# cscott/compressjs

Hardware: NVIDIA H100
Metric: bzip2_-9_encode_MBps (higher is better)
Workload: dtype u8

## Files before the change

compressjs_b200/csrc/huff.cu:

```cuda
#include "enc.h"
#include "huffalloc.cuh"

#define HF_THREADS 256
#define HF_TILE_GROUPS 256
#define HF_TILE_BYTES (HF_TILE_GROUPS * HUFF_GROUP)
#define HF_TILE_VEC (HF_TILE_BYTES / 16)
#define HF_TILE_REGS ((HF_TILE_VEC + HF_THREADS - 1) / HF_THREADS)
#define HF_COPIES 16
#define HF_EVEN 0x01F07C1Fu

struct HuffSmem {
  u8 tile[HF_TILE_BYTES + 16];
  u16 cost[SEL_STRIDE];
  u8 sel[SEL_STRIDE];
  u32 tbl[HUFF_MAXSYM][HF_COPIES];
  u32 freq[HUFF_MAXGROUPS][HUFF_MAXSYM + 2];
  int work[HUFF_MAXGROUPS][HUFF_MAXSYM + 2];
  u32 skey[HUFF_MAXGROUPS][HUFF_MAXSYM + 2];
  u16 order[HUFF_MAXGROUPS][HUFF_MAXSYM + 2];
  u8 len[HUFF_MAXGROUPS][HUFF_MAXSYM + 6];
  u32 chist[1024];
  u32 ws[HF_THREADS / 32 + 1];
  u32 gcount[HUFF_MAXGROUPS];
  u32 misc[8];
};

template <class S>
__device__ void pack_lengths(S& s, u32 ntab, u32 A) {
  for (u32 i = threadIdx.x; i < A * HF_COPIES; i += HF_THREADS) {
    const u32 sym = i / HF_COPIES;
    u32 p = 0;
    for (u32 t = 0; t < ntab; t++) p |= (u32)s.len[t][sym] << (5 * t);
    s.tbl[sym][i % HF_COPIES] = p;
  }
  __syncthreads();
}

__device__ void build_tables(HuffSmem& s, u32 ntab, u32 A) {
  const u32 tid = threadIdx.x;
  for (u32 i = tid; i < ntab * A; i += HF_THREADS) {
    const u32 t = i / A, sym = i % A;
    s.skey[t][sym] = (s.freq[t][sym] << 9) | sym;
  }
  __syncthreads();
  for (u32 i = tid; i < ntab * A; i += HF_THREADS) {
    const u32 t = i / A, sym = i % A;
    const u32 k = s.skey[t][sym];
    u32 r = 0;
    for (u32 j = 0; j < A; j++) r += (s.skey[t][j] < k) ? 1u : 0u;
    s.order[t][r] = (u16)sym;
    s.work[t][r] = (int)(k >> 9);
  }
  __syncthreads();
  if (tid < ntab) ha_allocate(s.work[tid], (int)A, 20);
  __syncthreads();
  for (u32 i = tid; i < ntab * A; i += HF_THREADS) {
    const u32 t = i / A, r = i % A;
    s.len[t][s.order[t][r]] = (u8)s.work[t][r];
  }
  __syncthreads();
  pack_lengths(s, ntab, A);
}

struct TileRegs {
  uint4 r[HF_TILE_REGS];
  unsigned long long hm;
};
__device__ __forceinline__ void tile_fetch(TileRegs& t, const u8* nar, const unsigned long long* hmask, u32 g0, u32 nsel, bool any_hi) {
  const uint4* src = reinterpret_cast<const uint4*>(nar + (size_t)g0 * HUFF_GROUP);
#pragma unroll
  for (int k = 0; k < HF_TILE_REGS; k++) {
    const u32 i = k * HF_THREADS + threadIdx.x;
    if (i < HF_TILE_VEC) t.r[k] = __ldg(src + i);
  }
  t.hm = any_hi && g0 + threadIdx.x < nsel ? __ldg(hmask + g0 + threadIdx.x) : 0ull;
}
__device__ __forceinline__ void tile_store(const TileRegs& t, u8* tile) {
#pragma unroll
  for (int k = 0; k < HF_TILE_REGS; k++) {
    const u32 i = k * HF_THREADS + threadIdx.x;
    if (i < HF_TILE_VEC) reinterpret_cast<uint4*>(tile)[i] = t.r[k];
  }
}

template <class F>
__device__ __forceinline__ void for_group(const u8* tile, u32 cnt, unsigned long long hm, F f) {
  const u32 base = threadIdx.x * HUFF_GROUP;
  if (cnt == HUFF_GROUP && hm == 0) {
    const u32* wp = reinterpret_cast<const u32*>(tile + (base & ~3u));
    const u32 sh = (base & 2u) * 8u;
    u32 nxt = wp[0];
#pragma unroll
    for (u32 k = 0; k < 13; k++) {
      const u32 cur = nxt;
      nxt = wp[k + 1];
      const u32 w = __funnelshift_r(cur, nxt, sh);
      f(w & 0xffu);
      f((w >> 8) & 0xffu);
      if (k < 12) {
        f((w >> 16) & 0xffu);
        f(w >> 24);
      }
    }
  } else {
    for (u32 j = 0; j < cnt; j++) f((u32)tile[base + j] | (u32)((hm >> j) & 1u) << 8);
  }
}

template <class S>
__device__ __forceinline__ void assign_selectors(S& s, const u8* nar, const unsigned long long* hmask, u32 m, u32 nsel, u32 ntab,
                                                 bool any_hi) {
  const u32 tid = threadIdx.x, lane = tid % HF_COPIES;
  TileRegs tr;
  tile_fetch(tr, nar, hmask, 0, nsel, any_hi);
  for (u32 g0 = 0; g0 < nsel; g0 += HF_TILE_GROUPS) {
    tile_store(tr, s.tile);
    const unsigned long long hm = tr.hm;
    __syncthreads();
    if (g0 + HF_TILE_GROUPS < nsel) tile_fetch(tr, nar, hmask, g0 + HF_TILE_GROUPS, nsel, any_hi);
    const u32 g = g0 + tid;
    if (g < nsel) {
      const u32 cnt = min(50u, m - 50u * g);
      u32 ae = 0, ao = 0;
      for_group(s.tile, cnt, hm, [&](u32 sy) {
        const u32 v = s.tbl[sy][lane];
        ae += v & HF_EVEN;
        ao += (v >> 5) & HF_EVEN;
      });
      const u32 c[HUFF_MAXGROUPS] = {ae & 1023u, ao & 1023u, (ae >> 10) & 1023u, (ao >> 10) & 1023u, ae >> 20, ao >> 20};
      u32 best = 0, bc = c[0];
#pragma unroll
      for (u32 t = 1; t < HUFF_MAXGROUPS; t++)
        if (t < ntab && c[t] < bc) { best = t; bc = c[t]; }
      s.sel[g] = (u8)best;
      s.cost[g] = (u16)bc;
    }
    __syncthreads();
  }
}

template <class S>
__device__ __forceinline__ void recount(S& s, const u8* nar, const unsigned long long* hmask, u32 m, u32 nsel, u32 ntab, bool any_hi) {
  const u32 tid = threadIdx.x;
  for (u32 i = tid; i < ntab * (HUFF_MAXSYM + 2); i += HF_THREADS) (&s.freq[0][0])[i] = 0;
  TileRegs tr;
  tile_fetch(tr, nar, hmask, 0, nsel, any_hi);
  __syncthreads();
  for (u32 g0 = 0; g0 < nsel; g0 += HF_TILE_GROUPS) {
    tile_store(tr, s.tile);
    const unsigned long long hm = tr.hm;
    __syncthreads();
    if (g0 + HF_TILE_GROUPS < nsel) tile_fetch(tr, nar, hmask, g0 + HF_TILE_GROUPS, nsel, any_hi);
    const u32 g = g0 + tid;
    if (g < nsel) {
      u32* f = s.freq[s.sel[g]];
      for_group(s.tile, min(50u, m - 50u * g), hm, [&](u32 sy) { atomicAdd(&f[sy], 1u); });
    }
    __syncthreads();
  }
}

__device__ __forceinline__ u32 mtf6_find(u32 list, u32 v) {
  u32 j = 0;
#pragma unroll
  for (u32 k = 1; k < HUFF_MAXGROUPS; k++) j = (((list >> (4 * k)) & 15u) == v) ? k : j;
  return j;
}
__device__ __forceinline__ u32 mtf6_front(u32 list, u32 j) {
  const u32 v = (list >> (4 * j)) & 15u;
  const u32 low = list & ((1u << (4 * j)) - 1u);
  const u32 high = list & ~((1u << (4 * (j + 1))) - 1u);
  return high | (low << 4) | v;
}
__device__ __forceinline__ u32 rec_apply(u32 R, u32 v) {
  u32 cnt = R >> 28, lst = R & 0x00ffffffu, j = cnt;
#pragma unroll
  for (u32 k = 0; k < HUFF_MAXGROUPS; k++) j = (k < cnt && ((lst >> (4 * k)) & 15u) == v) ? k : j;
  if (j == cnt) {
    lst = ((lst << 4) | v) & 0x00ffffffu;
    cnt++;
  } else {
    const u32 low = lst & ((1u << (4 * j)) - 1u);
    const u32 high = lst & ~((1u << (4 * (j + 1))) - 1u);
    lst = high | (low << 4) | v;
  }
  return (cnt << 28) | lst;
}
__device__ __forceinline__ bool rec_has(u32 R, u32 v) {
  const u32 cnt = R >> 28;
  bool f = false;
#pragma unroll
  for (u32 k = 0; k < HUFF_MAXGROUPS; k++) f = f || (k < cnt && ((R >> (4 * k)) & 15u) == v);
  return f;
}
__device__ __forceinline__ u32 rec_op(u32 A, u32 B) {
  u32 cnt = B >> 28, lst = B & 0x00ffffffu;
  const u32 ca = A >> 28;
#pragma unroll
  for (u32 k = 0; k < HUFF_MAXGROUPS; k++) {
    const u32 v = (A >> (4 * k)) & 15u;
    if (k < ca && !rec_has(B, v)) { lst |= v << (4 * cnt); cnt++; }
  }
  return (cnt << 28) | lst;
}
__device__ __forceinline__ u32 rec_full(u32 R) {
  u32 cnt = R >> 28, lst = R & 0x00ffffffu;
#pragma unroll
  for (u32 v = 0; v < HUFF_MAXGROUPS; v++)
    if (!rec_has(R, v)) { lst |= v << (4 * cnt); cnt++; }
  return lst;
}

template <class S>
__device__ void write_block(S& s, u32 blk, u32 m, u32 alpha, u32 nsel, u32 ng, const u32* __restrict__ used, u8* __restrict__ sel_out,
                            u8* __restrict__ selmtf_out, HuffBlk* __restrict__ hb, u32* __restrict__ goff_out) {
  const u32 tid = threadIdx.x, A = alpha + 2;
  unsigned long long bits;
  {
    const u32 w = tid >> 5, lane = tid & 31;
    const u32 per = (nsel + HF_THREADS / 32 - 1) / (HF_THREADS / 32);
    const u32 ga = min(nsel, w * per), gb = min(nsel, ga + per);
    u32 part = 0;
    for (u32 g = ga + lane; g < gb; g += 32) part += s.cost[g];
    part = warp_reduce_add(part);
    if (lane == 0) s.ws[w] = part;
    __syncthreads();
    u32 carry = 0, total = 0;
    for (u32 i = 0; i < HF_THREADS / 32; i++) {
      const u32 x = s.ws[i];
      carry += i < w ? x : 0u;
      total += x;
    }
    u32* go = goff_out + (size_t)blk * SEL_STRIDE;
    for (u32 g0 = ga; g0 < gb; g0 += 32) {
      const u32 g = g0 + lane;
      const u32 c = g < gb ? (u32)s.cost[g] : 0u;
      const u32 inc = warp_incl_add(c);
      if (g < gb) go[g] = carry + inc - c;
      carry += __shfl_sync(FULL_MASK, inc, 31);
    }
    if (tid == 0) go[nsel] = total;
    bits = total;
    __syncthreads();
  }
  u8* so = sel_out + (size_t)blk * SEL_STRIDE;
  for (u32 g = tid; g < nsel; g += HF_THREADS) so[g] = s.sel[g];
  for (u32 i = tid; i < ng * A; i += HF_THREADS) hb->len[i / A][i % A] = s.len[i / A][i % A];
  u32 selbits = 0;
  {
    const u32 per = (nsel + HF_THREADS - 1) / HF_THREADS;
    const u32 ga = min(nsel, tid * per), gb = min(nsel, ga + per);
    u32 P = 0;
    for (u32 g = ga; g < gb; g++) P = rec_apply(P, s.sel[g]);
    u32* sa = s.chist;
    u32* sb = s.chist + HF_THREADS;
    sa[tid] = P;
    __syncthreads();
    u32 *src = sa, *dst = sb;
    for (u32 o = 1; o < HF_THREADS; o <<= 1) {
      u32 x = src[tid];
      if (tid >= o) x = rec_op(src[tid - o], x);
      dst[tid] = x;
      __syncthreads();
      u32* tmp = src; src = dst; dst = tmp;
    }
    u32 L = rec_full(tid ? src[tid - 1] : 0u);
    u8* sm = selmtf_out + (size_t)blk * SEL_STRIDE;
    for (u32 g = ga; g < gb; g++) {
      const u32 j = mtf6_find(L, s.sel[g]);
      L = mtf6_front(L, j);
      sm[g] = (u8)j;
      selbits += j + 1;
    }
    __syncthreads();
  }
  {
    unsigned long long b2 = selbits;
    __shared__ unsigned long long red2[HF_THREADS / 32];
    for (int o = 16; o > 0; o >>= 1) b2 += __shfl_xor_sync(FULL_MASK, b2, o);
    if ((tid & 31) == 0) red2[tid >> 5] = b2;
    __syncthreads();
    b2 = 0;
    for (int i = 0; i < HF_THREADS / 32; i++) b2 += red2[i];
    bits += b2;
  }
  if (tid == 0) {
    unsigned long long hbits = 48 + 32 + 1 + 24 + 16 + 3 + 15;
    for (u32 r = 0; r < 16; r++) {
      const u32 w = used[blk * 8 + (r >> 1)];
      if ((w >> ((r & 1) * 16)) & 0xffffu) hbits += 16;
    }
    for (u32 t = 0; t < ng; t++) {
      hbits += 5;
      u32 cur = s.len[t][0];
      for (u32 i = 0; i < A; i++) {
        const u32 l = s.len[t][i];
        hbits += 2 * (l > cur ? l - cur : cur - l) + 1;
        cur = l;
      }
    }
    hb->ngroups = ng; hb->nsel = nsel; hb->alpha = alpha; hb->m = m;
    hb->body_bits = hbits + bits;
  }
}

__global__ void __launch_bounds__(HF_THREADS, 2)
k_huffman(const u8* __restrict__ sym_lo, const unsigned long long* __restrict__ sym_hi, const u32* __restrict__ any_hi_arr,
          const u32* __restrict__ m_arr, const u32* __restrict__ freq0, const u32* __restrict__ used, u8* __restrict__ sel_out,
          u8* __restrict__ selmtf_out, HuffBlk* __restrict__ hb_out, u32* __restrict__ goff_out) {
  extern __shared__ __align__(16) unsigned char smem_raw[];
  HuffSmem& s = *reinterpret_cast<HuffSmem*>(smem_raw);
  const u32 tid = threadIdx.x;
  const u32 blk = blockIdx.x;
  const u32 m = m_arr[blk];
  HuffBlk* hb = hb_out + blk;
  if (m == 0) {
    if (tid == 0) { hb->ngroups = 0; hb->nsel = 0; hb->alpha = 0; hb->m = 0; hb->body_bits = 0; }
    return;
  }
  u32 alpha = 0;
  for (int k = 0; k < 8; k++) alpha += __popc(used[blk * 8 + k]);
  const u32 A = alpha + 2;
  const u32 nsel = (m + HUFF_GROUP - 1) / HUFF_GROUP;
  const u8* nar = sym_lo + ((size_t)blk << SEG_SHIFT);
  const unsigned long long* hmask = sym_hi + (size_t)blk * SEL_STRIDE;
  const bool any_hi = any_hi_arr[blk] != 0;
  u32 target;
  if (m >= 2400) target = 6; else if (m >= 1200) target = 5; else if (m >= 600) target = 4; else if (m >= 200) target = 3; else target = 2;
  for (u32 i = tid; i < A; i += HF_THREADS) { s.freq[0][i] = freq0[(size_t)blk * HUFF_MAXSYM + i]; s.freq[1][i] = 1; }
  __syncthreads();
  u32 ng = 2;
  build_tables(s, ng, A);
  while (ng < target) {
    assign_selectors(s, nar, hmask, m, nsel, ng, any_hi);
    if (tid < HUFF_MAXGROUPS) s.gcount[tid] = 0;
    for (u32 i = tid; i < 1024; i += HF_THREADS) s.chist[i] = 0;
    __syncthreads();
    {
      u32 l0 = 0, l1 = 0, l2 = 0, l3 = 0, l4 = 0, l5 = 0;
      for (u32 g = tid; g < nsel; g += HF_THREADS) {
        const u32 v = s.sel[g];
        l0 += v == 0; l1 += v == 1; l2 += v == 2; l3 += v == 3; l4 += v == 4; l5 += v == 5;
      }
      if (l0) atomicAdd(&s.gcount[0], l0);
      if (l1) atomicAdd(&s.gcount[1], l1);
      if (l2) atomicAdd(&s.gcount[2], l2);
      if (l3) atomicAdd(&s.gcount[3], l3);
      if (l4) atomicAdd(&s.gcount[4], l4);
      if (l5) atomicAdd(&s.gcount[5], l5);
    }
    __syncthreads();
    u32 which = 0;
    for (u32 t = 1; t < ng; t++) if (s.gcount[t] > s.gcount[which]) which = t;
    const u32 cntw = s.gcount[which];
    for (u32 g = tid; g < nsel; g += HF_THREADS) if (s.sel[g] == which) atomicAdd(&s.chist[s.cost[g]], 1u);
    __syncthreads();
    if (tid == 0) {
      const u32 half = cntw >> 1;
      u32 cum = 0, cstar = 0;
      for (u32 cv = 0; cv < 1024; cv++) {
        if (cum + s.chist[cv] > half) { cstar = cv; break; }
        cum += s.chist[cv];
      }
      s.misc[0] = cstar;
      s.misc[1] = half - cum;
    }
    __syncthreads();
    const u32 cstar = s.misc[0], keep_eq = s.misc[1];
    {
      const u32 per = (nsel + HF_THREADS - 1) / HF_THREADS;
      const u32 ga = tid * per, gb = min(nsel, ga + per);
      u32 eq = 0;
      for (u32 g = ga; g < gb; g++) eq += (s.sel[g] == which && s.cost[g] == cstar) ? 1u : 0u;
      u32 tot;
      u32 ex = block_excl_add<HF_THREADS, u32>(eq, s.ws, &tot);
      for (u32 g = ga; g < gb; g++) {
        if (s.sel[g] != which) continue;
        const u32 cg = s.cost[g];
        bool move;
        if (cg > cstar) move = true;
        else if (cg < cstar) move = false;
        else { move = ex >= keep_eq; ex++; }
        if (move) s.sel[g] = (u8)ng;
      }
    }
    __syncthreads();
    ng++;
    recount(s, nar, hmask, m, nsel, ng, any_hi);
    build_tables(s, ng, A);
  }
  assign_selectors(s, nar, hmask, m, nsel, ng, any_hi);
  write_block(s, blk, m, alpha, nsel, ng, used, sel_out, selmtf_out, hb, goff_out);
}

struct LbHeap {
  u32 weight[2 * HUFF_MAXSYM];
  u16 parent[2 * HUFF_MAXSYM];
  u16 heap[HUFF_MAXSYM + 2];
};
#define LB_ROOT 0xffffu
#define LB_MAXLEN 17
struct HuffSmemL {
  u8 tile[HF_TILE_BYTES + 16];
  u16 cost[SEL_STRIDE];
  u8 sel[SEL_STRIDE];
  u32 tbl[HUFF_MAXSYM][HF_COPIES];
  u32 freq[HUFF_MAXGROUPS][HUFF_MAXSYM + 2];
  u8 len[HUFF_MAXGROUPS][HUFF_MAXSYM + 6];
  union {
    LbHeap hp[HUFF_MAXGROUPS];
    u32 chist[2 * HF_THREADS];
  };
  u32 ws[HF_THREADS / 32 + 1];
};
static_assert(sizeof(HuffSmemL) + 64 <= 115 * 1024, "two libbz2 Huffman CTAs per SM");

__device__ __forceinline__ void lb_up(LbHeap& h, u32 z) {
  const u32 tmp = h.heap[z];
  while (h.weight[tmp] < h.weight[h.heap[z >> 1]]) { h.heap[z] = h.heap[z >> 1]; z >>= 1; }
  h.heap[z] = (u16)tmp;
}
__device__ __forceinline__ void lb_down(LbHeap& h, u32 z, u32 nHeap) {
  const u32 tmp = h.heap[z];
  for (;;) {
    u32 y = z << 1;
    if (y > nHeap) break;
    if (y < nHeap && h.weight[h.heap[y + 1]] < h.weight[h.heap[y]]) y++;
    if (h.weight[tmp] < h.weight[h.heap[y]]) break;
    h.heap[z] = h.heap[y];
    z = y;
  }
  h.heap[z] = (u16)tmp;
}
__device__ void lb_make_lengths(LbHeap& h, const u32* freq, u8* len, u32 A) {
  for (u32 i = 0; i < A; i++) h.weight[i + 1] = (freq[i] ? freq[i] : 1u) << 8;
  for (;;) {
    u32 nNodes = A, nHeap = 0;
    h.heap[0] = 0; h.weight[0] = 0;
    for (u32 i = 1; i <= A; i++) {
      h.parent[i] = LB_ROOT;
      h.heap[++nHeap] = (u16)i;
      lb_up(h, nHeap);
    }
    while (nHeap > 1) {
      const u32 n1 = h.heap[1];
      h.heap[1] = h.heap[nHeap--];
      lb_down(h, 1, nHeap);
      const u32 n2 = h.heap[1];
      h.heap[1] = h.heap[nHeap--];
      lb_down(h, 1, nHeap);
      nNodes++;
      h.parent[n1] = h.parent[n2] = (u16)nNodes;
      const u32 w1 = h.weight[n1], w2 = h.weight[n2];
      h.weight[nNodes] = ((w1 & 0xffffff00u) + (w2 & 0xffffff00u)) | (1u + max(w1 & 0xffu, w2 & 0xffu));
      h.parent[nNodes] = LB_ROOT;
      h.heap[++nHeap] = (u16)nNodes;
      lb_up(h, nHeap);
    }
    bool too_long = false;
    for (u32 i = 1; i <= A; i++) {
      u32 j = 0;
      for (u32 k = i; h.parent[k] != LB_ROOT; k = h.parent[k]) j++;
      len[i - 1] = (u8)j;
      too_long |= j > LB_MAXLEN;
    }
    if (!too_long) return;
    for (u32 i = 1; i <= A; i++) h.weight[i] = (1u + (h.weight[i] >> 8) / 2) << 8;
  }
}

__device__ void cost_selected(HuffSmemL& s, const u8* nar, const unsigned long long* hmask, u32 m, u32 nsel, bool any_hi) {
  const u32 tid = threadIdx.x, lane = tid % HF_COPIES;
  TileRegs tr;
  tile_fetch(tr, nar, hmask, 0, nsel, any_hi);
  for (u32 g0 = 0; g0 < nsel; g0 += HF_TILE_GROUPS) {
    tile_store(tr, s.tile);
    const unsigned long long hm = tr.hm;
    __syncthreads();
    if (g0 + HF_TILE_GROUPS < nsel) tile_fetch(tr, nar, hmask, g0 + HF_TILE_GROUPS, nsel, any_hi);
    const u32 g = g0 + tid;
    if (g < nsel) {
      const u32 sh = 5 * s.sel[g];
      u32 c = 0;
      for_group(s.tile, min(50u, m - 50u * g), hm, [&](u32 sy) { c += (s.tbl[sy][lane] >> sh) & 31u; });
      s.cost[g] = (u16)c;
    }
    __syncthreads();
  }
}

__global__ void __launch_bounds__(HF_THREADS, 2)
k_huffman_libbz2(const u8* __restrict__ sym_lo, const unsigned long long* __restrict__ sym_hi, const u32* __restrict__ any_hi_arr,
                 const u32* __restrict__ m_arr, const u32* __restrict__ freq0, const u32* __restrict__ used, u8* __restrict__ sel_out,
                 u8* __restrict__ selmtf_out, HuffBlk* __restrict__ hb_out, u32* __restrict__ goff_out) {
  extern __shared__ __align__(16) unsigned char smem_raw[];
  HuffSmemL& s = *reinterpret_cast<HuffSmemL*>(smem_raw);
  const u32 tid = threadIdx.x;
  const u32 blk = blockIdx.x;
  const u32 m = m_arr[blk];
  HuffBlk* hb = hb_out + blk;
  if (m == 0) {
    if (tid == 0) { hb->ngroups = 0; hb->nsel = 0; hb->alpha = 0; hb->m = 0; hb->body_bits = 0; }
    return;
  }
  u32 alpha = 0;
  for (int k = 0; k < 8; k++) alpha += __popc(used[blk * 8 + k]);
  const u32 A = alpha + 2;
  const u32 nsel = (m + HUFF_GROUP - 1) / HUFF_GROUP;
  const u8* nar = sym_lo + ((size_t)blk << SEG_SHIFT);
  const unsigned long long* hmask = sym_hi + (size_t)blk * SEL_STRIDE;
  const bool any_hi = any_hi_arr[blk] != 0;
  u32 ng;
  if (m < 200) ng = 2; else if (m < 600) ng = 3; else if (m < 1200) ng = 4; else if (m < 2400) ng = 5; else ng = 6;
  if (tid == 0) {
    const u32* mf = freq0 + (size_t)blk * HUFF_MAXSYM;
    u32 remF = m, gs = 0;
    for (u32 nPart = ng; nPart > 0; nPart--) {
      const u32 tFreq = remF / nPart;
      int ge = (int)gs - 1;
      u32 aFreq = 0;
      while (aFreq < tFreq && ge < (int)A - 1) aFreq += mf[++ge];
      if (ge > (int)gs && nPart != ng && nPart != 1 && ((ng - nPart) & 1)) aFreq -= mf[ge--];
      for (u32 v = 0; v < A; v++) s.len[nPart - 1][v] = ((int)v >= (int)gs && (int)v <= ge) ? 0 : 15;
      gs = (u32)(ge + 1);
      remF -= aFreq;
    }
  }
  __syncthreads();
  pack_lengths(s, ng, A);
  for (int it = 0; it < 4; it++) {
    assign_selectors(s, nar, hmask, m, nsel, ng, any_hi);
    recount(s, nar, hmask, m, nsel, ng, any_hi);
    if (tid < ng) lb_make_lengths(s.hp[tid], s.freq[tid], s.len[tid], A);
    __syncthreads();
    pack_lengths(s, ng, A);
  }
  cost_selected(s, nar, hmask, m, nsel, any_hi);
  write_block(s, blk, m, alpha, nsel, ng, used, sel_out, selmtf_out, hb, goff_out);
}

void huffman_batch(Ctx& c, const NarrowSyms& sym, const u32* d_m, const u32* d_freq, const u32* d_used, u32 nblk, u8* d_sel, u8* d_selmtf,
                   HuffBlk* d_hb, u32* d_goff) {
  static bool attr = false;
  if (!attr) {
    CUDA_CHECK(cudaFuncSetAttribute(k_huffman, cudaFuncAttributeMaxDynamicSharedMemorySize, (int)sizeof(HuffSmem)));
    CUDA_CHECK(cudaFuncSetAttribute(k_huffman_libbz2, cudaFuncAttributeMaxDynamicSharedMemorySize, (int)sizeof(HuffSmemL)));
    attr = true;
  }
  if (c.bz_flavor == B2_BZ2_LIBBZ2) {
    k_huffman_libbz2<<<nblk, HF_THREADS, sizeof(HuffSmemL), c.stream>>>(sym.lo, sym.hi, sym.any_hi, d_m, d_freq, d_used, d_sel, d_selmtf, d_hb,
                                                                        d_goff);
    KLAUNCH(c); KCHECK();
    return;
  }
  k_huffman<<<nblk, HF_THREADS, sizeof(HuffSmem), c.stream>>>(sym.lo, sym.hi, sym.any_hi, d_m, d_freq, d_used, d_sel, d_selmtf, d_hb, d_goff);
  KLAUNCH(c); KCHECK();
}
```

Before: 26440.

## Stream Huffman symbol tiles via TMA bulk copies into an mbarrier ring

Replaces the register-staged tile prefetch with a multi-stage ring of bulk global-to-shared copies tracked by mbarriers. Each thread handles one group per stage, so two stages are consumed per step. This overlaps loads with the selector, recount and cost passes and frees registers. Shared memory is reorganised so the ring is unioned with the scratch arrays. The diff also batches the odd-field accumulation, uses byte_perm for byte extraction, and adds optional clock64 phase stamps. The risks are the stricter shared-memory budget, an over-read past the segment end, and mbarrier parity correctness across repeated passes.

```diff
diff --git a/compressjs_b200/csrc/huff.cu b/compressjs_b200/csrc/huff.cu
--- a/compressjs_b200/csrc/huff.cu
+++ b/compressjs_b200/csrc/huff.cu
@@ -1,29 +1,60 @@
 #include "enc.h"
 #include "huffalloc.cuh"
+#include "tma.cuh"
 
 #define HF_THREADS 256
-#define HF_TILE_GROUPS 256
-#define HF_TILE_BYTES (HF_TILE_GROUPS * HUFF_GROUP)
-#define HF_TILE_VEC (HF_TILE_BYTES / 16)
-#define HF_TILE_REGS ((HF_TILE_VEC + HF_THREADS - 1) / HF_THREADS)
+#define HF_STAGE_GROUPS 128
+#define HF_STAGE_BYTES (HF_STAGE_GROUPS * HUFF_GROUP)
+#define HF_STAGE_STRIDE (HF_STAGE_BYTES + 16)
+#define HF_STEP_STAGES (HF_THREADS / HF_STAGE_GROUPS)
+#ifndef HF_RING
+#define HF_RING 4
+#endif
 #define HF_COPIES 16
 #define HF_EVEN 0x01F07C1Fu
+#define HF_ODD (HF_EVEN << 5)
+static_assert(HF_RING >= HF_STEP_STAGES, "a step's stages fit in the ring");
+static_assert(((SEL_STRIDE + HF_STAGE_GROUPS - 1) / HF_STAGE_GROUPS) * HF_STAGE_BYTES <= SEG_SIZE, "ring over-read stays in the segment");
 
 struct HuffSmem {
-  u8 tile[HF_TILE_BYTES + 16];
+  union {
+    alignas(16) u8 ring[HF_RING][HF_STAGE_STRIDE];
+    struct {
+      int work[HUFF_MAXGROUPS][HUFF_MAXSYM + 2];
+      u32 skey[HUFF_MAXGROUPS][HUFF_MAXSYM + 2];
+      u16 order[HUFF_MAXGROUPS][HUFF_MAXSYM + 2];
+    };
+    u32 chist[1024];
+  };
+  u64 bar[HF_RING];
   u16 cost[SEL_STRIDE];
   u8 sel[SEL_STRIDE];
   u32 tbl[HUFF_MAXSYM][HF_COPIES];
   u32 freq[HUFF_MAXGROUPS][HUFF_MAXSYM + 2];
-  int work[HUFF_MAXGROUPS][HUFF_MAXSYM + 2];
-  u32 skey[HUFF_MAXGROUPS][HUFF_MAXSYM + 2];
-  u16 order[HUFF_MAXGROUPS][HUFF_MAXSYM + 2];
   u8 len[HUFF_MAXGROUPS][HUFF_MAXSYM + 6];
-  u32 chist[1024];
   u32 ws[HF_THREADS / 32 + 1];
   u32 gcount[HUFF_MAXGROUPS];
   u32 misc[8];
 };
+static_assert(sizeof(HuffSmem) + 64 <= 113 * 1024, "two Huffman CTAs per SM");
+
+#ifdef HF_STAMPS
+enum { HS_ASSIGN, HS_RECOUNT, HS_BUILD, HS_SPLIT, HS_WRITE, HS_BLOCKS, HS_N };
+__device__ unsigned long long hf_stamp[HS_N];
+#define HF_STAMP_INIT long long hs_last = clock64(), hs_acc[HS_BLOCKS] = {};
+#define HF_STAMP(p) do { if (threadIdx.x == 0) { const long long t = clock64(); hs_acc[p] += t - hs_last; hs_last = t; } } while (0)
+#define HF_STAMP_DONE                                                                              \
+  do {                                                                                             \
+    if (threadIdx.x == 0) {                                                                        \
+      for (int p = 0; p < HS_BLOCKS; p++) atomicAdd(&hf_stamp[p], (unsigned long long)hs_acc[p]);  \
+      atomicAdd(&hf_stamp[HS_BLOCKS], 1ull);                                                       \
+    }                                                                                              \
+  } while (0)
+#else
+#define HF_STAMP_INIT
+#define HF_STAMP(p) do {} while (0)
+#define HF_STAMP_DONE do {} while (0)
+#endif
 
 template <class S>
 __device__ void pack_lengths(S& s, u32 ntab, u32 A) {
@@ -62,30 +93,37 @@
   pack_lengths(s, ntab, A);
 }
 
-struct TileRegs {
-  uint4 r[HF_TILE_REGS];
-  unsigned long long hm;
-};
-__device__ __forceinline__ void tile_fetch(TileRegs& t, const u8* nar, const unsigned long long* hmask, u32 g0, u32 nsel, bool any_hi) {
-  const uint4* src = reinterpret_cast<const uint4*>(nar + (size_t)g0 * HUFF_GROUP);
-#pragma unroll
-  for (int k = 0; k < HF_TILE_REGS; k++) {
-    const u32 i = k * HF_THREADS + threadIdx.x;
-    if (i < HF_TILE_VEC) t.r[k] = __ldg(src + i);
-  }
-  t.hm = any_hi && g0 + threadIdx.x < nsel ? __ldg(hmask + g0 + threadIdx.x) : 0ull;
-}
-__device__ __forceinline__ void tile_store(const TileRegs& t, u8* tile) {
-#pragma unroll
-  for (int k = 0; k < HF_TILE_REGS; k++) {
-    const u32 i = k * HF_THREADS + threadIdx.x;
-    if (i < HF_TILE_VEC) reinterpret_cast<uint4*>(tile)[i] = t.r[k];
-  }
+template <class S, class F>
+__device__ __forceinline__ void stream_groups(S& s, u32& pos, const u8* nar, const unsigned long long* hmask, u32 m, u32 nsel, bool any_hi,
+                                              F f) {
+  const u32 tid = threadIdx.x, nst = (nsel + HF_STAGE_GROUPS - 1) / HF_STAGE_GROUPS, p0 = pos;
+  auto issue = [&](u32 q) {
+    const u32 slot = (p0 + q) % HF_RING;
+    mbar_expect_tx(&s.bar[slot], HF_STAGE_BYTES);
+    bulk_g2s(s.ring[slot], nar + (size_t)q * HF_STAGE_BYTES, HF_STAGE_BYTES, &s.bar[slot]);
+  };
+  fence_async_smem();
+  __syncthreads();
+  if (tid == 0)
+    for (u32 q = 0; q < HF_RING && q < nst; q++) issue(q);
+  const u32 gi = tid % HF_STAGE_GROUPS, base = gi * HUFF_GROUP;
+  for (u32 q0 = 0; q0 < nst; q0 += HF_STEP_STAGES) {
+    const u32 q = q0 + tid / HF_STAGE_GROUPS, g = q * HF_STAGE_GROUPS + gi;
+    if (g < nsel) {
+      const unsigned long long hm = any_hi ? __ldg(hmask + g) : 0ull;
+      const u32 G = p0 + q;
+      mbar_wait(&s.bar[G % HF_RING], (G / HF_RING) & 1u);
+      f(g, s.ring[G % HF_RING], base, min(50u, m - 50u * g), hm);
+    }
+    __syncthreads();
+    if (tid == 0)
+      for (u32 q = q0 + HF_RING; q < q0 + HF_RING + HF_STEP_STAGES && q < nst; q++) issue(q);
+  }
+  pos = p0 + nst;
 }
 
 template <class F>
-__device__ __forceinline__ void for_group(const u8* tile, u32 cnt, unsigned long long hm, F f) {
-  const u32 base = threadIdx.x * HUFF_GROUP;
+__device__ __forceinline__ void for_group(const u8* tile, u32 base, u32 cnt, unsigned long long hm, F f) {
   if (cnt == HUFF_GROUP && hm == 0) {
     const u32* wp = reinterpret_cast<const u32*>(tile + (base & ~3u));
     const u32 sh = (base & 2u) * 8u;
@@ -95,11 +133,11 @@
       const u32 cur = nxt;
       nxt = wp[k + 1];
       const u32 w = __funnelshift_r(cur, nxt, sh);
-      f(w & 0xffu);
-      f((w >> 8) & 0xffu);
+      f(__byte_perm(w, 0, 0x4440));
+      f(__byte_perm(w, 0, 0x4441));
       if (k < 12) {
-        f((w >> 16) & 0xffu);
-        f(w >> 24);
+        f(__byte_perm(w, 0, 0x4442));
+        f(__byte_perm(w, 0, 0x4443));
       }
     }
   } else {
@@ -108,56 +146,35 @@
 }
 
 template <class S>
-__device__ __forceinline__ void assign_selectors(S& s, const u8* nar, const unsigned long long* hmask, u32 m, u32 nsel, u32 ntab,
+__device__ __forceinline__ void assign_selectors(S& s, u32& pos, const u8* nar, const unsigned long long* hmask, u32 m, u32 nsel, u32 ntab,
                                                  bool any_hi) {
-  const u32 tid = threadIdx.x, lane = tid % HF_COPIES;
-  TileRegs tr;
-  tile_fetch(tr, nar, hmask, 0, nsel, any_hi);
-  for (u32 g0 = 0; g0 < nsel; g0 += HF_TILE_GROUPS) {
-    tile_store(tr, s.tile);
-    const unsigned long long hm = tr.hm;
-    __syncthreads();
-    if (g0 + HF_TILE_GROUPS < nsel) tile_fetch(tr, nar, hmask, g0 + HF_TILE_GROUPS, nsel, any_hi);
-    const u32 g = g0 + tid;
-    if (g < nsel) {
-      const u32 cnt = min(50u, m - 50u * g);
-      u32 ae = 0, ao = 0;
-      for_group(s.tile, cnt, hm, [&](u32 sy) {
-        const u32 v = s.tbl[sy][lane];
-        ae += v & HF_EVEN;
-        ao += (v >> 5) & HF_EVEN;
-      });
-      const u32 c[HUFF_MAXGROUPS] = {ae & 1023u, ao & 1023u, (ae >> 10) & 1023u, (ao >> 10) & 1023u, ae >> 20, ao >> 20};
-      u32 best = 0, bc = c[0];
-#pragma unroll
-      for (u32 t = 1; t < HUFF_MAXGROUPS; t++)
-        if (t < ntab && c[t] < bc) { best = t; bc = c[t]; }
-      s.sel[g] = (u8)best;
-      s.cost[g] = (u16)bc;
-    }
-    __syncthreads();
-  }
+  const u32* tl = &s.tbl[0][threadIdx.x % HF_COPIES];
+  stream_groups(s, pos, nar, hmask, m, nsel, any_hi, [&](u32 g, const u8* tile, u32 base, u32 cnt, unsigned long long hm) {
+    u32 ae = 0, ao = 0, to = 0, k = 0;
+    for_group(tile, base, cnt, hm, [&](u32 sy) {
+      const u32 v = tl[sy * HF_COPIES];
+      ae += v & HF_EVEN;
+      to += v & HF_ODD;
+      if (++k == 4) { ao += to >> 5; to = 0; k = 0; }
+    });
+    ao += to >> 5;
+    const u32 c[HUFF_MAXGROUPS] = {ae & 1023u, ao & 1023u, (ae >> 10) & 1023u, (ao >> 10) & 1023u, ae >> 20, ao >> 20};
+    u32 best = 0, bc = c[0];
+#pragma unroll
+    for (u32 t = 1; t < HUFF_MAXGROUPS; t++)
+      if (t < ntab && c[t] < bc) { best = t; bc = c[t]; }
+    s.sel[g] = (u8)best;
+    s.cost[g] = (u16)bc;
+  });
 }
 
 template <class S>
-__device__ __forceinline__ void recount(S& s, const u8* nar, const unsigned long long* hmask, u32 m, u32 nsel, u32 ntab, bool any_hi) {
-  const u32 tid = threadIdx.x;
-  for (u32 i = tid; i < ntab * (HUFF_MAXSYM + 2); i += HF_THREADS) (&s.freq[0][0])[i] = 0;
-  TileRegs tr;
-  tile_fetch(tr, nar, hmask, 0, nsel, any_hi);
-  __syncthreads();
-  for (u32 g0 = 0; g0 < nsel; g0 += HF_TILE_GROUPS) {
-    tile_store(tr, s.tile);
-    const unsigned long long hm = tr.hm;
-    __syncthreads();
-    if (g0 + HF_TILE_GROUPS < nsel) tile_fetch(tr, nar, hmask, g0 + HF_TILE_GROUPS, nsel, any_hi);
-    const u32 g = g0 + tid;
-    if (g < nsel) {
-      u32* f = s.freq[s.sel[g]];
-      for_group(s.tile, min(50u, m - 50u * g), hm, [&](u32 sy) { atomicAdd(&f[sy], 1u); });
-    }
-    __syncthreads();
-  }
+__device__ __forceinline__ void recount(S& s, u32& pos, const u8* nar, const unsigned long long* hmask, u32 m, u32 nsel, u32 ntab, bool any_hi) {
+  for (u32 i = threadIdx.x; i < ntab * (HUFF_MAXSYM + 2); i += HF_THREADS) (&s.freq[0][0])[i] = 0;
+  stream_groups(s, pos, nar, hmask, m, nsel, any_hi, [&](u32 g, const u8* tile, u32 base, u32 cnt, unsigned long long hm) {
+    u32* f = s.freq[s.sel[g]];
+    for_group(tile, base, cnt, hm, [&](u32 sy) { atomicAdd(&f[sy], 1u); });
+  });
 }
 
 __device__ __forceinline__ u32 mtf6_find(u32 list, u32 v) {
@@ -327,12 +344,20 @@
   const bool any_hi = any_hi_arr[blk] != 0;
   u32 target;
   if (m >= 2400) target = 6; else if (m >= 1200) target = 5; else if (m >= 600) target = 4; else if (m >= 200) target = 3; else target = 2;
+  HF_STAMP_INIT
+  if (tid == 0) {
+    for (u32 i = 0; i < HF_RING; i++) mbar_init(&s.bar[i], 1);
+    mbar_fence_init();
+  }
+  u32 pos = 0;
   for (u32 i = tid; i < A; i += HF_THREADS) { s.freq[0][i] = freq0[(size_t)blk * HUFF_MAXSYM + i]; s.freq[1][i] = 1; }
   __syncthreads();
   u32 ng = 2;
   build_tables(s, ng, A);
+  HF_STAMP(HS_BUILD);
   while (ng < target) {
-    assign_selectors(s, nar, hmask, m, nsel, ng, any_hi);
+    assign_selectors(s, pos, nar, hmask, m, nsel, ng, any_hi);
+    HF_STAMP(HS_ASSIGN);
     if (tid < HUFF_MAXGROUPS) s.gcount[tid] = 0;
     for (u32 i = tid; i < 1024; i += HF_THREADS) s.chist[i] = 0;
     __syncthreads();
@@ -386,11 +411,17 @@
     }
     __syncthreads();
     ng++;
-    recount(s, nar, hmask, m, nsel, ng, any_hi);
+    HF_STAMP(HS_SPLIT);
+    recount(s, pos, nar, hmask, m, nsel, ng, any_hi);
+    HF_STAMP(HS_RECOUNT);
     build_tables(s, ng, A);
-  }
-  assign_selectors(s, nar, hmask, m, nsel, ng, any_hi);
+    HF_STAMP(HS_BUILD);
+  }
+  assign_selectors(s, pos, nar, hmask, m, nsel, ng, any_hi);
+  HF_STAMP(HS_ASSIGN);
   write_block(s, blk, m, alpha, nsel, ng, used, sel_out, selmtf_out, hb, goff_out);
+  HF_STAMP(HS_WRITE);
+  HF_STAMP_DONE;
 }
 
 struct LbHeap {
@@ -401,19 +432,20 @@
 #define LB_ROOT 0xffffu
 #define LB_MAXLEN 17
 struct HuffSmemL {
-  u8 tile[HF_TILE_BYTES + 16];
+  union {
+    alignas(16) u8 ring[HF_RING][HF_STAGE_STRIDE];
+    LbHeap hp[HUFF_MAXGROUPS];
+    u32 chist[2 * HF_THREADS];
+  };
+  u64 bar[HF_RING];
   u16 cost[SEL_STRIDE];
   u8 sel[SEL_STRIDE];
   u32 tbl[HUFF_MAXSYM][HF_COPIES];
   u32 freq[HUFF_MAXGROUPS][HUFF_MAXSYM + 2];
   u8 len[HUFF_MAXGROUPS][HUFF_MAXSYM + 6];
-  union {
-    LbHeap hp[HUFF_MAXGROUPS];
-    u32 chist[2 * HF_THREADS];
-  };
   u32 ws[HF_THREADS / 32 + 1];
 };
-static_assert(sizeof(HuffSmemL) + 64 <= 115 * 1024, "two libbz2 Huffman CTAs per SM");
+static_assert(sizeof(HuffSmemL) + 64 <= 113 * 1024, "two libbz2 Huffman CTAs per SM");
 
 __device__ __forceinline__ void lb_up(LbHeap& h, u32 z) {
   const u32 tmp = h.heap[z];
@@ -469,24 +501,17 @@
   }
 }
 
-__device__ void cost_selected(HuffSmemL& s, const u8* nar, const unsigned long long* hmask, u32 m, u32 nsel, bool any_hi) {
-  const u32 tid = threadIdx.x, lane = tid % HF_COPIES;
-  TileRegs tr;
-  tile_fetch(tr, nar, hmask, 0, nsel, any_hi);
-  for (u32 g0 = 0; g0 < nsel; g0 += HF_TILE_GROUPS) {
-    tile_store(tr, s.tile);
-    const unsigned long long hm = tr.hm;
-    __syncthreads();
-    if (g0 + HF_TILE_GROUPS < nsel) tile_fetch(tr, nar, hmask, g0 + HF_TILE_GROUPS, nsel, any_hi);
-    const u32 g = g0 + tid;
-    if (g < nsel) {
-      const u32 sh = 5 * s.sel[g];
-      u32 c = 0;
-      for_group(s.tile, min(50u, m - 50u * g), hm, [&](u32 sy) { c += (s.tbl[sy][lane] >> sh) & 31u; });
-      s.cost[g] = (u16)c;
-    }
-    __syncthreads();
-  }
+__device__ void cost_selected(HuffSmemL& s, u32& pos, const u8* nar, const unsigned long long* hmask, u32 m, u32 nsel, bool any_hi) {
+  const u32* tl = &s.tbl[0][threadIdx.x % HF_COPIES];
+  stream_groups(s, pos, nar, hmask, m, nsel, any_hi, [&](u32 g, const u8* tile, u32 base, u32 cnt, unsigned long long hm) {
+    const u32 sh = 5 * s.sel[g], mask = 31u << sh;
+    u32 c = 0, t = 0, k = 0;
+    for_group(tile, base, cnt, hm, [&](u32 sy) {
+      t += tl[sy * HF_COPIES] & mask;
+      if (++k == 4) { c += t >> sh; t = 0; k = 0; }
+    });
+    s.cost[g] = (u16)(c + (t >> sh));
+  });
 }
 
 __global__ void __launch_bounds__(HF_THREADS, 2)
@@ -513,6 +538,11 @@
   u32 ng;
   if (m < 200) ng = 2; else if (m < 600) ng = 3; else if (m < 1200) ng = 4; else if (m < 2400) ng = 5; else ng = 6;
   if (tid == 0) {
+    for (u32 i = 0; i < HF_RING; i++) mbar_init(&s.bar[i], 1);
+    mbar_fence_init();
+  }
+  u32 pos = 0;
+  if (tid == 0) {
     const u32* mf = freq0 + (size_t)blk * HUFF_MAXSYM;
     u32 remF = m, gs = 0;
     for (u32 nPart = ng; nPart > 0; nPart--) {
@@ -529,13 +559,13 @@
   __syncthreads();
   pack_lengths(s, ng, A);
   for (int it = 0; it < 4; it++) {
-    assign_selectors(s, nar, hmask, m, nsel, ng, any_hi);
-    recount(s, nar, hmask, m, nsel, ng, any_hi);
+    assign_selectors(s, pos, nar, hmask, m, nsel, ng, any_hi);
+    recount(s, pos, nar, hmask, m, nsel, ng, any_hi);
     if (tid < ng) lb_make_lengths(s.hp[tid], s.freq[tid], s.len[tid], A);
     __syncthreads();
     pack_lengths(s, ng, A);
   }
-  cost_selected(s, nar, hmask, m, nsel, any_hi);
+  cost_selected(s, pos, nar, hmask, m, nsel, any_hi);
   write_block(s, blk, m, alpha, nsel, ng, used, sel_out, selmtf_out, hb, goff_out);
 }
 
@@ -555,4 +585,12 @@
   }
   k_huffman<<<nblk, HF_THREADS, sizeof(HuffSmem), c.stream>>>(sym.lo, sym.hi, sym.any_hi, d_m, d_freq, d_used, d_sel, d_selmtf, d_hb, d_goff);
   KLAUNCH(c); KCHECK();
-}
+#ifdef HF_STAMPS
+  unsigned long long st[HS_N];
+  CUDA_CHECK(cudaMemcpyFromSymbolAsync(st, hf_stamp, sizeof(st), 0, cudaMemcpyDeviceToHost, c.stream));
+  CUDA_CHECK(cudaStreamSynchronize(c.stream));
+  const double nb = st[HS_BLOCKS] ? (double)st[HS_BLOCKS] : 1.0;
+  fprintf(stderr, "hf_stamps blocks=%llu kcycles/block assign=%.1f recount=%.1f build=%.1f split=%.1f write=%.1f\n", st[HS_BLOCKS],
+          st[HS_ASSIGN] / nb / 1e3, st[HS_RECOUNT] / nb / 1e3, st[HS_BUILD] / nb / 1e3, st[HS_SPLIT] / nb / 1e3, st[HS_WRITE] / nb / 1e3);
+#endif
+}
```

Result: no change. 26780, median of 6 (+1.3%).
